# ygjwd12345/UCD

Measured on AMD Instinct MI355X. Metric: images/sec (whole node) per UCD train step, VOC 15-5 step-1, 513^2 bs=24, higher is better.
Workload: dtype bf16

## Files before the change

### include/ucd_hip.h

```cpp
#ifndef UCD_HIP_H
#define UCD_HIP_H

#include <stddef.h>
#include <stdint.h>

#ifdef __cplusplus
extern "C" {
#endif

#define UCD_VERSION 100

typedef void* ucd_stream_t;
typedef void* ucd_comm_t;

enum ucd_dtype { UCD_F32 = 0, UCD_BF16 = 1 };
enum ucd_act { UCD_ACT_IDENTITY = 0, UCD_ACT_LEAKY_RELU = 1, UCD_ACT_ELU = 2  };
#define UCD_ACT_MASK 0xff
#define UCD_NORM_ABS_GAMMA 0x100
enum ucd_pixcon_precision { UCD_PIXCON_F32 = 0, UCD_PIXCON_F16 = 1, UCD_PIXCON_F16_SPLIT = 2 };
enum ucd_error {
  UCD_OK = 0,
  UCD_EINVAL = -1,
  UCD_EALIGN = -2,
  UCD_EWORKSPACE = -3,
// ... 193 lines not shown
                            const int32_t* anchor_pix, const ucd_pixcon_meta* meta,
                            const float* grad_scale, void* d_f_n, int ld_d, int dtype, int BHW, int N,
                            ucd_stream_t stream);

enum ucd_seg_form {
  UCD_SEG_PK_16_8 = 1,
  UCD_SEG_PK_20_4 = 2,
  UCD_SEG_PK_12_12 = 3,
  UCD_SEG_REG_24_16 = 4,
  UCD_SEG_REG_24_24 = 5,
  UCD_SEG_WIDE_FIXED = 6,
  UCD_SEG_WIDE_F32 = 7
};
int ucd_seg_losses_plan(int H, int W, int h, int w, int Ctot, int K, int has_teacher, int d_sem_aligned, int pk, int* form,
                        int* ny, int* nx, size_t* lds_bytes);
size_t ucd_seg_losses_workspace_bytes(int B, int H, int W);
int ucd_seg_losses(const float* sem_s, int ld_s, const float* sem_t, int ld_t, const int64_t* labels,
                   int B, int H, int W, int h, int w, int Ctot, int K, int ignore_index,
                   float ce_weight, float kd_weight, float* loss_out, float* d_sem, int ld_d,
                   void* workspace, size_t workspace_bytes, ucd_stream_t stream);

enum ucd_seg_kd_mode { UCD_KD_UNBIASED = 0, UCD_KD_PLAIN = 1 };
int ucd_seg_losses_plan_ex(int H, int W, int h, int w, int Ctot, int K, int ce_old_cl, int kd_mode, int has_teacher,
                           int d_sem_aligned, int pk, int* form, int* ny, int* nx, size_t* lds_bytes);
int ucd_seg_losses_ex(const float* sem_s, int ld_s, const float* sem_t, int ld_t, const int64_t* labels,
                      int B, int H, int W, int h, int w, int Ctot, int K, int ce_old_cl, int kd_mode, float alpha,
                      int ignore_index, float ce_weight, float kd_weight, float* loss_out, float* d_sem, int ld_d,
                      void* workspace, size_t workspace_bytes, ucd_stream_t stream);

int ucd_seg_confusion(const float* sem, int ld_s, const int64_t* labels, int B, int H, int W, int h, int w, int Ctot,
                      int n_classes, int64_t* hist, int64_t* pred, ucd_stream_t stream);

int ucd_label_path(const uint8_t* const* src, const int* desc, int B, int S, const uint8_t* lut, int* tables,
                   int64_t* out, ucd_stream_t stream);

int ucd_image_path(const uint8_t* const* src, const int* desc, int B, int S, int kmax, int hmax, float mean_r, float mean_g,
                   float mean_b, float std_r, float std_g, float std_b, int* coeff_ws, uint8_t* tmp, float* out,
                   ucd_stream_t stream);

typedef struct ucd_conv1x1_desc {
  const void* a;  int lda;
  const void* w;  int ldw;
  void* y;        int ldy;
  int M, N, K;
  const float* in_mean;  const float* in_scale;  const float* in_shift;  int in_act;  float in_slope;
  int out_mode;
  const float* out_mean;  const float* out_scale;  const float* out_shift;  const float* out_invstd;
  const void* residual;  int ldr;
  int out_act;  float out_slope;
  float* partial;
  int accumulate;
  int taps, H, W, dilation;
  const void* side2;  int ld2;
  int stride;
  float* stat_acc;  const float* stat_shift;  float* stat_acc2;
  int stat_rep;
} ucd_conv1x1_desc;

int ucd_conv1x1_row_tiles(int M);
int ucd_conv1x1_stat_replicas(int M);
size_t ucd_conv1x1_stats_partial_bytes(int M, int C);
int ucd_conv1x1(const ucd_conv1x1_desc* desc, ucd_stream_t stream);

int ucd_conv1x1_stats_finalize(const float* partial, int M, int C, const float* weight, float* running_mean,
                               float* running_var, float momentum, float eps, float* buf, float* pack, int flags,
                               ucd_stream_t stream);

int ucd_abn_reduce_partials(const float* partial, int tiles, int C, float* sums, float* sums_copy, const float* weight,
                            int flags, ucd_stream_t stream);

size_t ucd_conv1x1_wgrad_workspace_bytes(int M, int N, int K);
int ucd_conv1x1_wgrad(const void* dy, int ld_dy, const void* a, int lda, int M, int N, int K,
                      const float* in_mean, const float* in_scale, const float* in_shift, int in_act, float in_slope,
                      void* dw, void* workspace, size_t workspace_bytes, ucd_stream_t stream);

int ucd_abn_sync_finalize(const float* gathered, int world, int M, int C, const float* weight, float* running_mean,
                          float* running_var, float momentum, float eps, float* buf, int flags, ucd_stream_t stream);

int ucd_stem_conv7x7(const float* x, long long sb, long long sc, long long sh, long long sw, int B, int H, int W, const void* w,
                     void* z, ucd_stream_t stream);

int ucd_stem_conv_pool(const float* x, long long sb, long long sc, long long sh, long long sw, int B, int H, int W, const void* w,
                       const float* mean, const float* scale, const float* beta, int act, float slope, void* out, ucd_stream_t stream);
int ucd_stem_pooled_size(int n);
size_t ucd_stem_pool_workspace_bytes(int C);
int ucd_stem_apply_pool(const void* z, int B, int H, int W, int C, const float* mean, const float* scale, const float* beta, int act,
                        float slope, void* out, uint8_t* idx, ucd_stream_t stream);
int ucd_stem_pool_backward(const void* z, const void* dpool, const uint8_t* idx, int B, int H, int W, int C, const float* mean,
                           const float* invstd, const float* scale, const float* beta, const float* weight, float* sums, float count,
                           int act, float slope, void* dz, void* workspace, size_t workspace_bytes, int phase, ucd_stream_t stream);

size_t ucd_conv_wgrad_workspace_bytes(int M, int N, int K, int taps);
int ucd_conv_wgrad(const void* dz, int ld_dz, const void* x, int ld_x, int M, int N, int K, int taps, int H, int W, int dilation,
                   void* dw, float* dw32, int accumulate32, void* workspace, size_t workspace_bytes, ucd_stream_t stream);
int ucd_conv_wgrad_strided(const void* dz, int ld_dz, const void* x, int ld_x, int M, int N, int K, int taps, int H, int W,
                           int dilation, int stride, void* dw, float* dw32, int accumulate32, void* workspace, size_t workspace_bytes,
                           ucd_stream_t stream);
int ucd_conv_wgrad_ex(const void* dz, int ld_dz, const void* x, int ld_x, int M, int N, int K, int taps, int H, int W, int dilation,
                      int stride, void* dw, float* dw32, int accumulate32, void* workspace, size_t workspace_bytes, int flags,
                      ucd_stream_t stream);
int ucd_conv_wgrad_defer(int mode);
int ucd_conv_wgrad_mode(void);
int ucd_conv_wgrad_flush(ucd_stream_t stream);
int ucd_conv_wgrad_drop(ucd_stream_t stream);
int ucd_conv_wgrad_drop_all(void);

int ucd_flip_weights_batched(const void* src_flat, void* dst_flat, const int* blocks, int n_blocks, const long long* entries,
                             ucd_stream_t stream);
int ucd_flip_weights_batched64(const void* src_flat, void* dst_flat, const int* blocks, int n_blocks, const long long* entries,
                               ucd_stream_t stream);

int ucd_transpose_bf16(const void* src, int rows, int cols, void* dst, ucd_stream_t stream);

int ucd_conv_f32(const float* a, int lda, const float* w, int ldw, float* y, int ldy, int M, int N, int K, int taps, int H, int W,
                 int dilation, int accumulate, ucd_stream_t stream);
size_t ucd_conv_f32_wgrad_workspace_bytes(int M, int N, int K, int taps);
int ucd_conv_f32_wgrad(const float* dz, int ld_dz, const float* x, int ld_x, int M, int N, int K, int taps, int H, int W,
                       int dilation, float* dw, void* workspace, size_t workspace_bytes, ucd_stream_t stream);

#define UCD_SGD_MAX_GROUPS 8
typedef struct ucd_sgd_tensor {
  float* p;  const float* g;  float* m;  void* w16;
  long long n;
  int group;  int pad;
} ucd_sgd_tensor;
typedef struct ucd_sgd_hyper {
  double lr[UCD_SGD_MAX_GROUPS], momentum[UCD_SGD_MAX_GROUPS], weight_decay[UCD_SGD_MAX_GROUPS];
  int nesterov[UCD_SGD_MAX_GROUPS];
} ucd_sgd_hyper;
int ucd_sgd_chunk(void);
int ucd_sgd_step(const ucd_sgd_tensor* table, const int* blocks, int n_blocks, const ucd_sgd_hyper* hyper, ucd_stream_t stream);
int ucd_sgd_hyper_store(ucd_sgd_hyper* device_hyper, const ucd_sgd_hyper* hyper, ucd_stream_t stream);
int ucd_sgd_step_dev(const ucd_sgd_tensor* table, const int* blocks, int n_blocks, const ucd_sgd_hyper* device_hyper,
                     ucd_stream_t stream);

#define UCD_REG_EWC 0
#define UCD_REG_PI 1
#define UCD_REG_RW 2
typedef struct ucd_reg_tensor {
  float* p;  float* g;  const float* p_old;  const float* omega;
  float* fisher;  float* score;  float* temp;
  long long n;
  int penalize;  int pad;
} ucd_reg_tensor;
typedef struct ucd_reg_hyper {
  double reg_importance;
  float alpha, one_minus_alpha, lambda_f;
  int iterations;
  int counter;
  int pad;
} ucd_reg_hyper;
int ucd_reg_chunk(void);
int ucd_reg_hyper_store(ucd_reg_hyper* device_hyper, const ucd_reg_hyper* hyper, ucd_stream_t stream);
int ucd_reg_step(const ucd_reg_tensor* table, const int* blocks, int n_blocks, int method, ucd_reg_hyper* device_hyper,
                 double* partials, float* penalty, ucd_stream_t stream);

#ifdef __cplusplus
}
#endif
#endif
```

### ucd_amd/backbone.py

```python
from __future__ import annotations

import sys
from collections import OrderedDict
from functools import partial

import torch
import torch.nn as nn

from . import switches as _switches
from .blocks import Conv2d, ResidualBlock, try_index

_STAGE_DILATION = {16: (1, 1, 1, 2), 8: (1, 1, 2, 4)}


class GlobalAvgPool2d(nn.Module):

    def forward(self, inputs):
        return inputs.flatten(2).mean(dim=2)


class ResNet(nn.Module):
    def __init__(self, structure, bottleneck, norm_act=nn.BatchNorm2d, classes=0,
                 output_stride=16, keep_outputs=False):
        super().__init__()
        if len(structure) != 4:
            raise ValueError("Expected a structure with four values")
        if output_stride not in _STAGE_DILATION:
            raise ValueError("Output stride must be 8 or 16")
        self.structure, self.bottleneck, self.keep_outputs = structure, bottleneck, keep_outputs
        self.dilation = dilation = list(_STAGE_DILATION[output_stride])

        stem = [("conv1", Conv2d(3, 64, 7, stride=2, padding=3, bias=False)), ("bn1", norm_act(64))]
        if try_index(dilation, 0) == 1:
            stem.append(("pool1", nn.MaxPool2d(3, stride=2, padding=1)))
        self.mod1 = nn.Sequential(OrderedDict(stem))

        width = (64, 64, 256) if bottleneck else (64, 64)
        cin = 64
        for stage, depth in enumerate(structure):
            d = try_index(dilation, stage)
            blocks = OrderedDict()
            for b in range(depth):
                stride = 2 if (d == 1 and b == 0 and stage > 0) else 1
                blocks[f"block{b + 1}"] = ResidualBlock(cin, width, norm_act=norm_act, stride=stride, dilation=d)
                cin = width[-1]
            self.add_module(f"mod{stage + 2}", nn.Sequential(blocks))
            width = tuple(2 * c for c in width)
        self.out_channels = cin

        if classes != 0:
            self.classifier = nn.Sequential(OrderedDict(
                [("avg_pool", GlobalAvgPool2d()), ("fc", nn.Linear(cin, classes))]))

    def _stem(self, x):
        m = self.mod1
        if hasattr(m, "pool1") and getattr(m.bn1, "ucd_fused_abn", False) and x.is_cuda:
            pool = m.pool1
            if (pool.kernel_size, pool.stride, pool.padding, pool.dilation, pool.ceil_mode) == (3, 2, 1, 1, False):
                from .abn import stem_norm_pool
                y = _stem_eval_fused(m.conv1, m.bn1, x)
                if y is not None:
                    return y
                z = _stem_conv(m.conv1, x)
                y = stem_norm_pool(m.bn1, z)
                return y if y is not None else pool(m.bn1(z))
        return m(x)

    def forward(self, x):
        outs = [self._stem(x)]
        for name in ("mod2", "mod3", "mod4", "mod5"):
            outs.append(getattr(self, name)(outs[-1]))
        if hasattr(self, "classifier"):
            outs.append(self.classifier(outs[-1]))
        return outs if self.keep_outputs else outs[-1]


class _StemConvFunction(torch.autograd.Function):

    @staticmethod
    def forward(ctx, x, w):
        from . import hip
        ctx.save_for_backward(x, w)
        return hip.stem_conv7x7(x, w)

    @staticmethod
    def backward(ctx, dz):
        x, w = ctx.saved_tensors
        dw = None
        if ctx.needs_input_grad[1]:
            xb = x.to(torch.bfloat16).contiguous(memory_format=torch.channels_last)
            dw = torch.ops.aten.convolution_backward(dz.contiguous(memory_format=torch.channels_last), xb, w, None, [2, 2], [3, 3],
                                                     [1, 1], False, [0, 0], 1, [False, True, False])[1]
        return None, dw


def _stem_conv(conv, x):
    w = conv.working_weight() if hasattr(conv, "working_weight") else None
    if w is None and x.is_cuda and torch.is_autocast_enabled() and torch.get_autocast_dtype("cuda") == torch.bfloat16:
        w = conv.weight.to(torch.bfloat16)
    if (w is None or not x.is_cuda or x.dim() != 4 or x.dtype != torch.float32 or x.requires_grad or conv.bias is not None
            or tuple(conv.weight.shape) != (64, 3, 7, 7) or conv.stride != (2, 2) or conv.padding != (3, 3)
            or conv.dilation != (1, 1) or w.dtype != torch.bfloat16 or not w.is_contiguous(memory_format=torch.channels_last)
            or _switches.get("UCD_OWN_STEM", "1") == "0"):
        return conv(x)
    if torch.is_grad_enabled() and w.requires_grad:
        return _StemConvFunction.apply(x, w)
    from . import hip
    return hip.stem_conv7x7(x, w)


def _stem_eval_fused(conv, bn, x):
    from . import abn as _abn
    if (torch.is_grad_enabled() or bn.training or _switches.get("UCD_STEM_EVAL_FUSED", "1") == "0" or _switches.get("UCD_OWN_STEM", "1") == "0"
            or _switches.get("UCD_STEM_FOLD", "1") == "0" or not getattr(bn, "ucd_fused_abn", False)
            or bn.activation not in ("leaky_relu", "identity")):
        return None
    w = conv.working_weight() if hasattr(conv, "working_weight") else None
    if w is None and x.is_cuda and torch.is_autocast_enabled() and torch.get_autocast_dtype("cuda") == torch.bfloat16:
        w = conv.weight.to(torch.bfloat16)
    if (w is None or not x.is_cuda or x.dim() != 4 or x.dtype != torch.float32 or conv.bias is not None
            or tuple(conv.weight.shape) != (64, 3, 7, 7) or conv.stride != (2, 2) or conv.padding != (3, 3) or conv.dilation != (1, 1)
            or w.dtype != torch.bfloat16 or not w.is_contiguous(memory_format=torch.channels_last) or x.shape[2] < 8 or x.shape[3] < 8):
        return None
    from . import hip
    invstd, scale = bn._eval_constants()
    return hip.stem_conv_pool(x, w, bn.running_mean, scale, bn.bias, _abn._act_code(bn.activation), bn.activation_param)


_NETS = {
    "18": ([2, 2, 2, 2], False), "34": ([3, 4, 6, 3], False), "50": ([3, 4, 6, 3], True),
    "101": ([3, 4, 23, 3], True), "152": ([3, 8, 36, 3], True),
}
__all__ = ["ResNet"]
for _n, (_s, _b) in _NETS.items():
    setattr(sys.modules[__name__], f"net_resnet{_n}", partial(ResNet, structure=_s, bottleneck=_b))
    __all__.append(f"net_resnet{_n}")
```

### ucd_amd/csrc/stem.hip

```cpp
#include "common.h"

namespace ucd {
namespace {

typedef __hip_bfloat16 bf16;
constexpr int kThreads = 256;
constexpr int kRedBlocks = 1024;
constexpr int kApplyRows = 4;

__device__ __forceinline__ float leaky(float z, float slope) { return z > 0.f ? z : z * slope; }
__device__ __forceinline__ float bf16_round(float v) { return __bfloat162float(__float2bfloat16(v)); }

struct StemArgs {
  const bf16* z; int B, H, W, C, PH, PW;
  const float *mean, *scale, *beta, *invstd, *weight, *sums;
  float slope, inv_count;
  int abs_gamma, cg_shift;
};

__global__ __launch_bounds__(kThreads) void stem_apply_pool_kernel(StemArgs p, bf16* __restrict__ out, uint8_t* __restrict__ idx) {
  const int cgs = p.cg_shift, CG = 1 << cgs;
  const int t = blockIdx.x * kThreads + threadIdx.x;
  const int cg = t & (CG - 1), pw = t >> cgs, ph = blockIdx.y, b = blockIdx.z;
  if (pw >= p.PW) return;
// ... 360 lines not shown
    if (tid < kSIP) {
#pragma unroll
      for (int r = 0; r < kSIR; ++r) {
        const bf16 v = __float2bfloat16((premask >> r) & 1u ? pre[r] : 0.f);
        In[r * kSIP + tid] = *reinterpret_cast<const unsigned short*>(&v);
      }
    }
    __syncthreads();
    if (tile + (int)gridDim.x < p.ntiles) fetch(tile + gridDim.x);
    f32x16 acc[2][2];
#pragma unroll
    for (int a = 0; a < 2; ++a)
#pragma unroll
      for (int c = 0; c < 2; ++c)
#pragma unroll
        for (int r = 0; r < 16; ++r) acc[a][c][r] = 0.f;
#pragma unroll
    for (int s = 0; s < kSK / 16; ++s) {
      const int t0 = 2 * s, t1 = 2 * s + 1;
      const int ky = h ? (t1 / 3 > 6 ? 6 : t1 / 3) : t0 / 3, j0 = h ? 8 * (t1 % 3) : 8 * (t0 % 3);
      bf16x8 wf[2], pf[2];
#pragma unroll
      for (int c = 0; c < 2; ++c) wf[c] = *reinterpret_cast<const bf16x8*>(&Wl[(c * 32 + col) * kSWP + 16 * s + 8 * h]);
#pragma unroll
      for (int a = 0; a < 2; ++a) {
        const int orow = wave * 2 + a;
        const unsigned* src = reinterpret_cast<const unsigned*>(&In[(2 * orow + ky) * kSIP + 6 * col + j0]);
        union { unsigned u[4]; bf16x8 v; } f;
        f.u[0] = src[0]; f.u[1] = src[1]; f.u[2] = src[2]; f.u[3] = src[3];
        pf[a] = f.v;
      }
#pragma unroll
      for (int a = 0; a < 2; ++a)
#pragma unroll
        for (int c = 0; c < 2; ++c) acc[a][c] = __builtin_amdgcn_mfma_f32_32x32x16_bf16(wf[c], pf[a], acc[a][c], 0, 0, 0);
    }
    const int ox = ox0 + col;
#pragma unroll
    for (int a = 0; a < 2; ++a) {
      const int orow = wave * 2 + a, oy = oy0 + orow;
      const bool inside = (unsigned)oy < (unsigned)p.OH && (unsigned)ox < (unsigned)p.OW;
      unsigned short* dst = Tl + (orow * kSTW + col) * kFTP;
#pragma unroll
      for (int c = 0; c < 2; ++c)
#pragma unroll
        for (int g = 0; g < 4; ++g) {
          const int ch = c * 32 + 8 * g + 4 * h;
          const float4 mu = *reinterpret_cast<const float4*>(Pl + ch), sc = *reinterpret_cast<const float4*>(Pl + 64 + ch);
          const float4 sh = *reinterpret_cast<const float4*>(Pl + 128 + ch);
          const float m4[4] = {mu.x, mu.y, mu.z, mu.w}, s4[4] = {sc.x, sc.y, sc.z, sc.w}, b4[4] = {sh.x, sh.y, sh.z, sh.w};
          union { bf16 v[4]; uint2 u; } o;
#pragma unroll
          for (int e = 0; e < 4; ++e) {
            const float zq = bf16_round(acc[a][c][g * 4 + e]);
            o.v[e] = __float2bfloat16(leaky((zq - m4[e]) * s4[e] + b4[e], q.slope));
          }
          if (!inside) o.u = make_uint2(0xFF80FF80u, 0xFF80FF80u);
          *reinterpret_cast<uint2*>(dst + ch) = o.u;
        }
    }
    __syncthreads();
    for (int i = tid; i < kFPH * kFPW * 8; i += kThreads) {
      const int cg = i & 7, pp = i >> 3, pr = pp / kFPW, pc = pp - pr * kFPW;
      const int ph = (oy0 + 1) / 2 + pr, pw = (ox0 + 1) / 2 + pc;
      if (ph >= q.PH || pw >= q.PW) continue;
      float best[8];
#pragma unroll
      for (int e = 0; e < 8; ++e) best[e] = -INFINITY;
#pragma unroll
      for (int kh = 0; kh < 3; ++kh)
#pragma unroll
        for (int kw = 0; kw < 3; ++kw) {
          Vec<bf16> v;
          v.raw = *reinterpret_cast<const uint4*>(Tl + ((2 * pr + kh) * kSTW + 2 * pc + kw) * kFTP + cg * 8);
#pragma unroll
          for (int e = 0; e < 8; ++e) best[e] = fmaxf(best[e], v.get(e));
        }
      Vec<bf16> o;
#pragma unroll
      for (int e = 0; e < 8; ++e) o.set(e, best[e]);
      o.store(q.out + (((size_t)b * q.PH + ph) * q.PW + pw) * 64 + cg * 8);
    }
  }
}

bool stem_args_ok(const void* z, int B, int H, int W, int C) {
  return z && B > 0 && B < 65536 && H > 1 && H < 65536 && W > 1 && C >= 8 && (C & (C - 1)) == 0 && C <= 2048 && aligned16(z);
}

}
}

using namespace ucd;

extern "C" {

int ucd_stem_pooled_size(int n) { return (n + 2 - 3) / 2 + 1; }

size_t ucd_stem_pool_workspace_bytes(int C) { return (size_t)kRedBlocks * 2 * C * sizeof(float); }

int ucd_stem_apply_pool(const void* z, int B, int H, int W, int C, const float* mean, const float* scale, const float* beta, int act,
                        float slope, void* out, uint8_t* idx, ucd_stream_t stream) {
  static const char* fn = "ucd_stem_apply_pool";
  UCD_REQUIRE(stem_args_ok(z, B, H, W, C) && mean && scale && out && aligned16(out) && (!idx || (reinterpret_cast<uintptr_t>(idx) & 7) == 0),
              UCD_EINVAL, "%s: dense channels-last bf16 maps with a power-of-two channel count in 8..2048 expected", fn);
  const int a = act & UCD_ACT_MASK;
  UCD_REQUIRE(a != UCD_ACT_ELU, UCD_EUNSUPPORTED, "%s: leaky_relu / identity only (an elu stem keeps the separate passes)", fn);
  StemArgs p{};
  p.z = (const bf16*)z; p.B = B; p.H = H; p.W = W; p.C = C; p.PH = ucd_stem_pooled_size(H); p.PW = ucd_stem_pooled_size(W);
  p.mean = mean; p.scale = scale; p.beta = beta; p.slope = a == UCD_ACT_IDENTITY ? 1.f : slope;
  p.cg_shift = __builtin_ctz(C / 8);
  stem_apply_pool_kernel<<<dim3(ceil_div(p.PW * (C / 8), kThreads), p.PH, B), kThreads, 0, (hipStream_t)stream>>>(p, (bf16*)out, idx);
  return check_launch(fn);
}

int ucd_stem_conv7x7(const float* x, long long sb, long long sc, long long sh, long long sw, int B, int H, int W, const void* w,
                     void* z, ucd_stream_t stream) {
  static const char* fn = "ucd_stem_conv7x7";
  UCD_REQUIRE(x && w && z && B > 0 && H > 0 && W > 0 && aligned16(z) && (reinterpret_cast<uintptr_t>(w) & 1) == 0, UCD_EINVAL,
              "%s: bad arguments", fn);
  StemConvArgs p{};
  p.x = x; p.sb = sb; p.sc = sc; p.sh = sh; p.sw = sw; p.w = (const bf16*)w; p.z = (bf16*)z;
  p.B = B; p.H = H; p.W = W; p.OH = (H + 6 - 7) / 2 + 1; p.OW = (W + 6 - 7) / 2 + 1;
  p.tiles_y = ceil_div(p.OH, kSTH); p.tiles_x = ceil_div(p.OW, kSTW); p.ntiles = B * p.tiles_y * p.tiles_x;
  const int grid = p.ntiles < 768 ? p.ntiles : 768;
  stem_conv7x7_kernel<<<grid, kThreads, 0, (hipStream_t)stream>>>(p);
  return check_launch(fn);
}

int ucd_stem_conv_pool(const float* x, long long sb, long long sc, long long sh, long long sw, int B, int H, int W, const void* w,
                       const float* mean, const float* scale, const float* beta, int act, float slope, void* out, ucd_stream_t stream) {
  static const char* fn = "ucd_stem_conv_pool";
  UCD_REQUIRE(x && w && out && mean && scale && B > 0 && H > 0 && W > 0 && aligned16(out) && (reinterpret_cast<uintptr_t>(w) & 1) == 0 &&
              aligned16(mean) && aligned16(scale) && (!beta || aligned16(beta)), UCD_EINVAL, "%s: bad arguments", fn);
  const int a = act & UCD_ACT_MASK;
  UCD_REQUIRE(a != UCD_ACT_ELU && !(act & UCD_NORM_ABS_GAMMA), UCD_EUNSUPPORTED, "%s: leaky_relu / identity with given scale only", fn);
  StemFusedArgs q{};
  StemConvArgs& p = q.c;
  p.x = x; p.sb = sb; p.sc = sc; p.sh = sh; p.sw = sw; p.w = (const bf16*)w; p.z = nullptr;
  p.B = B; p.H = H; p.W = W; p.OH = (H + 6 - 7) / 2 + 1; p.OW = (W + 6 - 7) / 2 + 1;
  q.PH = ucd_stem_pooled_size(p.OH); q.PW = ucd_stem_pooled_size(p.OW);
  p.tiles_y = ceil_div(q.PH, kFPH); p.tiles_x = ceil_div(q.PW, kFPW); p.ntiles = B * p.tiles_y * p.tiles_x;
  q.mean = mean; q.scale = scale; q.beta = beta; q.slope = a == UCD_ACT_IDENTITY ? 1.f : slope; q.out = (bf16*)out;
  const size_t lds = (size_t)(64 * kSWP + kSIR * kSIP + kSTH * kSTW * kFTP) * 2 + 3 * 64 * 4;
  UCD_TRY_LDS(stem_conv_pool_kernel, 80 * 1024);
  const int grid = p.ntiles < 512 ? p.ntiles : 512;
  stem_conv_pool_kernel<<<grid, kThreads, lds, (hipStream_t)stream>>>(q);
  return check_launch(fn);
}

int ucd_stem_pool_backward(const void* z, const void* dpool, const uint8_t* idx, int B, int H, int W, int C, const float* mean,
                           const float* invstd, const float* scale, const float* beta, const float* weight, float* sums, float count,
                           int act, float slope, void* dz, void* workspace, size_t workspace_bytes, int phase, ucd_stream_t stream) {
  static const char* fn = "ucd_stem_pool_backward";
  UCD_REQUIRE(stem_args_ok(z, B, H, W, C) && dpool && idx && mean && invstd && scale && sums && aligned16(dpool), UCD_EINVAL,
              "%s: bad arguments", fn);
  UCD_REQUIRE(phase >= 1 && phase <= 3 && (!(phase & 2) || (dz && aligned16(dz) && count > 0.f)), UCD_EINVAL, "%s: bad phase / dz", fn);
  const int a = act & UCD_ACT_MASK;
  UCD_REQUIRE(a != UCD_ACT_ELU, UCD_EUNSUPPORTED, "%s: leaky_relu / identity only", fn);
  StemArgs p{};
  p.z = (const bf16*)z; p.B = B; p.H = H; p.W = W; p.C = C; p.PH = ucd_stem_pooled_size(H); p.PW = ucd_stem_pooled_size(W);
  p.mean = mean; p.scale = scale; p.beta = beta; p.invstd = invstd; p.weight = weight; p.sums = sums;
  p.slope = a == UCD_ACT_IDENTITY ? 1.f : slope; p.abs_gamma = (act & UCD_NORM_ABS_GAMMA) != 0;
  p.cg_shift = __builtin_ctz(C / 8);
  hipStream_t s = (hipStream_t)stream;
  if (phase & 1) {
    UCD_REQUIRE(workspace && workspace_bytes >= ucd_stem_pool_workspace_bytes(C), UCD_EWORKSPACE, "%s: workspace too small", fn);
    stem_pool_bwd_reduce_kernel<<<kRedBlocks, kThreads, kThreads * 16 * sizeof(float), s>>>(p, (const bf16*)dpool, idx, (float*)workspace);
    int rc = check_launch(fn);
    if (rc) return rc;
    stem_sum_partials_kernel<<<2 * C, kThreads, 0, s>>>((const float*)workspace, kRedBlocks, C, p.abs_gamma ? weight : nullptr, sums);
    rc = check_launch(fn);
    if (rc) return rc;
  }
  if (phase & 2) {
    p.inv_count = 1.f / count;
    stem_pool_bwd_apply_kernel<<<dim3(ceil_div(((W + 1) / 2) * (C / 8), kThreads), ceil_div(H, kApplyRows), B), kThreads, 0, s>>>(p, (const bf16*)dpool, idx, (bf16*)dz);
    return check_launch(fn);
  }
  return 0;
}

}
```

### ucd_amd/hip.py

```python
from __future__ import annotations

import ctypes as C
import os

import torch

_HERE = os.path.dirname(os.path.abspath(__file__))
LIB_PATH = os.path.join(_HERE, "libucd_hip.so")

F32, BF16 = 0, 1
ACT_IDENTITY, ACT_LEAKY_RELU, ACT_ELU = 0, 1, 2
ACT_CODES = {"identity": ACT_IDENTITY, "leaky_relu": ACT_LEAKY_RELU, "elu": ACT_ELU}
ACT_MASK = 0xFF
NORM_ABS_GAMMA = 0x100
PIX_TILE = 128
PIXCON_LD = 256
PIXCON_F32, PIXCON_F16, PIXCON_F16_SPLIT = 0, 1, 2
KD_UNBIASED, KD_PLAIN = 0, 1
SEG_FORMS = {1: "pk<16,8>", 2: "pk<20,4>", 3: "pk<12,12>", 4: "reg<24,16>", 5: "reg<24,24>", 6: "wide/fixed", 7: "wide/f32"}
PIXCON_PATHS = {1: "f32", 2: "f32/wide", 3: "f16/planned", 4: "f16/split"}
PIXCON_PRECISION = {"f32": PIXCON_F32, "fp32": PIXCON_F32, "f16": PIXCON_F16, "fp16": PIXCON_F16,
                    "f16_split": PIXCON_F16_SPLIT}


# ... 12 lines not shown
    _fields_ = [("a", C.c_void_p), ("lda", C.c_int), ("w", C.c_void_p), ("ldw", C.c_int), ("y", C.c_void_p), ("ldy", C.c_int),
                ("M", C.c_int), ("N", C.c_int), ("K", C.c_int),
                ("in_mean", C.c_void_p), ("in_scale", C.c_void_p), ("in_shift", C.c_void_p), ("in_act", C.c_int),
                ("in_slope", C.c_float), ("out_mode", C.c_int),
                ("out_mean", C.c_void_p), ("out_scale", C.c_void_p), ("out_shift", C.c_void_p), ("out_invstd", C.c_void_p),
                ("residual", C.c_void_p), ("ldr", C.c_int), ("out_act", C.c_int), ("out_slope", C.c_float),
                ("partial", C.c_void_p), ("accumulate", C.c_int),
                ("taps", C.c_int), ("H", C.c_int), ("W", C.c_int), ("dilation", C.c_int),
                ("side2", C.c_void_p), ("ld2", C.c_int), ("stride", C.c_int),
                ("stat_acc", C.c_void_p), ("stat_shift", C.c_void_p), ("stat_acc2", C.c_void_p), ("stat_rep", C.c_int)]


_p, _i, _f, _z = C.c_void_p, C.c_int, C.c_float, C.c_size_t
SIGNATURES = {
    "ucd_version": (_i, []),
    "ucd_last_error": (C.c_char_p, []),
    "ucd_abn_workspace_bytes": (_z, [_i, _i]),
    "ucd_abn_stats": (_i, [_p, _i, _i, _i, _i, _p, _i, _p, _p, _p, _z, _p]),
    "ucd_abn_stats_finalize": (_i, [_p, _i, _i, _i, _i, _p, _i, _p, _p, _p, _p, _p, _f, _f, _p, _p, _p, _i, _p, _z, _p]),
    "ucd_abn_finalize": (_i, [_p, _p, _f, _i, _p, _p, _p, _f, _f, _p, _p, _p, _i, _p]),
    "ucd_abn_eval_params": (_i, [_p, _p, _f, _i, _p, _p, _i, _p]),
    "ucd_abn_apply": (_i, [_p, _i, _p, _i, _p, _i, _i, _i, _i, _p, _i, _p, _p, _p, _i, _f, _p]),
    "ucd_conv1x1_stat_replicas": (_i, [_i]),
    "ucd_fill_zero": (_i, [_p, _z, _p]),
    "ucd_abn_apply_stats": (_i, [_p, _i, _p, _i, _p, _i, _i, _i, _p, _i, _p, _f, _p, _p, _p, _p, _f, _f, _p, _p, _p, _i, _f, _p]),
    "ucd_abn_bwd_apply_raw": (_i, [_p, _i, _p, _i, _p, _i, _p, _i, _p, _i, _i, _i, _p, _p, _p, _p, _p, _p, _p, _i, _p, _f, _i, _f, _p]),
    "ucd_abn_bwd_reduce": (_i, [_p, _i, _p, _i, _p, _i, _i, _i, _i, _p, _i, _p, _p, _p, _p, _p, _i, _f, _p, _p, _z, _p]),
    "ucd_label_path": (_i, [_p, _p, _i, _i, _p, _p, _p, _p]),
    "ucd_image_path": (_i, [_p, _p, _i, _i, _i, _i, _f, _f, _f, _f, _f, _f, _p, _p, _p, _p]),
    "ucd_gemm_load": (_i, [C.c_char_p]),
    "ucd_gemm_workspace_bytes": (_z, []),
    "ucd_gemm_bf16": (_i, [_i, _i, _i, _i, _p, _i, _p, _i, _p, _i, _p, _z, _i, _p]),
    "ucd_gemm_bf16_acc": (_i, [_i, _i, _i, _i, _p, _i, _p, _i, _p, _i, _p, _z, _p]),
    "ucd_gemm_has_plan": (_i, [_i, _i, _i, _i, _i, _i, _i]),
    "ucd_gemm_last_tuned_us": (_f, []),
    "ucd_gemm_last_candidates": (_i, []),
    "ucd_comm_load": (_i, [C.c_char_p]),
    "ucd_comm_unique_id": (_i, [_p, _z]),
    "ucd_comm_init": (_i, [_p, _z, _i, _i, C.POINTER(C.c_void_p)]),
    "ucd_comm_destroy": (_i, [_p]),
    "ucd_comm_all_gather": (_i, [_p, _p, _p, _z, _p]),
    "ucd_comm_all_reduce_sum": (_i, [_p, _p, _z, _p]),
    "ucd_comm_init_local": (_i, [_i, _i, C.POINTER(C.c_void_p)]),
    "ucd_comm_ipc_handle_bytes": (_z, []),
    "ucd_comm_ipc_create": (_i, [_p, _i, _i, _p]),
    "ucd_comm_ipc_connect": (_i, [_p, _p]),
    "ucd_comm_ipc_drop": (_i, [_p]),
    "ucd_comm_ipc_timeouts": (C.c_uint, [_p]),
    "ucd_abn_sync_forward_comm": (_i, [_p, _i, _p, _i, _p, _i, _p, _i, _i, _i, _i, _p, _i, _p, _p, _p, _p, _f, _f, _p, _i, _f,
                                       _p, _z, _p]),
    "ucd_abn_sync_backward_comm": (_i, [_p, _i, _p, _i, _p, _i, _p, _i, _p, _i, _p, _i, _i, _i, _i, _p, _i, _p, _p, _p, _p, _p,
                                        _p, _p, _i, _f, _p, _z, _p]),
    "ucd_abn_sync_stats": (_i, [_p, _i, _i, _i, _i, _p, _i, _p, _p, _p, _p, _z, _p]),
    "ucd_abn_sync_forward": (_i, [_p, _i, _p, _i, _p, _i, _i, _i, _i, _p, _i, _p, _i, _p, _p, _p, _p, _f, _f, _p, _i, _f, _p]),
    "ucd_abn_sync_bwd_reduce": (_i, [_p, _i, _p, _i, _p, _i, _i, _i, _i, _p, _i, _p, _p, _p, _p, _p, _i, _f, _p, _p, _p, _z, _p]),
    "ucd_abn_bwd_apply": (_i, [_p, _i, _p, _i, _p, _i, _p, _i, _p, _i, _i, _i, _i, _p, _i, _p, _p, _p, _p, _p, _p,
                               _f, _i, _i, _f, _p]),
    "ucd_abn_forward": (_i, [_p, _i, _p, _i, _p, _i, _i, _i, _i, _p, _i, _p, _p, _p, _p, _f, _f, _i, _p, _p, _i, _f, _p, _z, _p]),
    "ucd_abn_backward": (_i, [_p, _i, _p, _i, _p, _i, _p, _i, _p, _i, _i, _i, _i, _p, _i, _p, _p, _p, _p, _p, _p, _f, _i, _i,
                              _i, _f, _p, _z, _p]),
    "ucd_plane_sum": (_i, [_p, _i, _i, _i, _i, _i, _f, _p, _p]),
    "ucd_window_mean_workspace_bytes": (_z, [_i, _i, _i, _i, _i]),
    "ucd_window_mean": (_i, [_p, _i, _i, _i, _i, _i, _i, _i, _i, _p, _i, _p, _z, _p]),
    "ucd_attmap_workspace_bytes": (_z, [_i, _i]),
    "ucd_attmap": (_i, [_p, _i, _p, _i, _i, _i, _i, _i, _p, _z, _p]),
    "ucd_attn_mse_workspace_bytes": (_z, [_i, _i]),
    "ucd_attn_mse": (_i, [_p, _i, _p, _i, _i, _i, _i, _i, _f, _p, _p, _i, _p, _z, _p]),
    "ucd_conv1x1_row_tiles": (_i, [_i]),
    "ucd_conv1x1_stats_partial_bytes": (_z, [_i, _i]),
    "ucd_conv1x1": (_i, [C.POINTER(Conv1x1Desc), _p]),
    "ucd_conv1x1_stats_finalize": (_i, [_p, _i, _i, _p, _p, _p, _f, _f, _p, _p, _i, _p]),
    "ucd_abn_reduce_partials": (_i, [_p, _i, _i, _p, _p, _p, _i, _p]),
    "ucd_conv1x1_wgrad_workspace_bytes": (_z, [_i, _i, _i]),
    "ucd_conv1x1_wgrad": (_i, [_p, _i, _p, _i, _i, _i, _i, _p, _p, _p, _i, _f, _p, _p, _z, _p]),
    "ucd_abn_sync_finalize": (_i, [_p, _i, _i, _i, _p, _p, _p, _f, _f, _p, _i, _p]),
    "ucd_stem_pooled_size": (_i, [_i]),
    "ucd_stem_pool_workspace_bytes": (_z, [_i]),
    "ucd_stem_apply_pool": (_i, [_p, _i, _i, _i, _i, _p, _p, _p, _i, _f, _p, _p, _p]),
    "ucd_stem_pool_backward": (_i, [_p, _p, _p, _i, _i, _i, _i, _p, _p, _p, _p, _p, _p, _f, _i, _f, _p, _p, _z, _i, _p]),
    "ucd_conv_wgrad_workspace_bytes": (_z, [_i, _i, _i, _i]),
    "ucd_conv_wgrad": (_i, [_p, _i, _p, _i, _i, _i, _i, _i, _i, _i, _i, _p, _p, _i, _p, _z, _p]),
    "ucd_stem_conv7x7": (_i, [_p, C.c_longlong, C.c_longlong, C.c_longlong, C.c_longlong, _i, _i, _i, _p, _p, _p]),
    "ucd_stem_conv_pool": (_i, [_p, C.c_longlong, C.c_longlong, C.c_longlong, C.c_longlong, _i, _i, _i, _p, _p, _p, _p, _i, _f, _p, _p]),
    "ucd_conv_wgrad_strided": (_i, [_p, _i, _p, _i, _i, _i, _i, _i, _i, _i, _i, _i, _p, _p, _i, _p, _z, _p]),
    "ucd_conv_wgrad_ex": (_i, [_p, _i, _p, _i, _i, _i, _i, _i, _i, _i, _i, _i, _p, _p, _i, _p, _z, _i, _p]),
    "ucd_conv_wgrad_defer": (_i, [_i]),
    "ucd_conv_wgrad_mode": (_i, []),
    "ucd_conv_wgrad_flush": (_i, [_p]),
    "ucd_conv_wgrad_drop": (_i, [_p]),
    "ucd_conv_wgrad_drop_all": (_i, []),
    "ucd_transpose_bf16": (_i, [_p, _i, _i, _p, _p]),
    "ucd_conv_f32": (_i, [_p, _i, _p, _i, _p, _i, _i, _i, _i, _i, _i, _i, _i, _i, _p]),
    "ucd_conv_f32_wgrad_workspace_bytes": (_z, [_i, _i, _i, _i]),
    "ucd_conv_f32_wgrad": (_i, [_p, _i, _p, _i, _i, _i, _i, _i, _i, _i, _i, _p, _p, _z, _p]),
    "ucd_flip_weights_batched": (_i, [_p, _p, _p, _i, _p, _p]),
    "ucd_flip_weights_batched64": (_i, [_p, _p, _p, _i, _p, _p]),
    "ucd_sgd_chunk": (_i, []),
    "ucd_sgd_step": (_i, [_p, _p, _i, _p, _p]),
    "ucd_sgd_hyper_store": (_i, [_p, _p, _p]),
    "ucd_sgd_step_dev": (_i, [_p, _p, _i, _p, _p]),
    "ucd_reg_chunk": (_i, []),
    "ucd_reg_hyper_store": (_i, [_p, _p, _p]),
    "ucd_reg_step": (_i, [_p, _p, _i, _i, _p, _p, _p, _p]),
    "ucd_pixcon_prep_workspace_bytes": (_z, [_i, _i]),
    "ucd_pixcon_prep": (_i, [_p, _i, _i, _i, _i, _i, _i, _p, _i, _i, _i, _i, _p, _p, _p, _p, _p, _p, _z, _p]),
    "ucd_pixcon_gather": (_i, [_p, _i, _p, _i, _i, _i, _i, _p, _p, _p, _i, _p, _p, _i, _p, _i, _p, _p, _p, _p]),
    "ucd_pixcon_loss_workspace_bytes": (_z, [_i, _i, _i]),
    "ucd_pixcon_loss_plan": (_i, [_i, _i, _i, _i, _f, _p, _p, _p, _p, _p, _p, _p]),
    "ucd_pixcon_loss": (_i, [_p, _i, _i, _p, _p, _i, _i, _p, _p, _i, _p, _i, _f, _i, _i, _p, _p, _i, _p, _p, _z, _p]),
    "ucd_pixcon_loss_given_p": (_i, [_p, _i, _i, _p, _p, _i, _p, _i, _f, _i, _p, _p, _i, _p, _p, _z, _p]),
    "ucd_pixcon_scatter_grad": (_i, [_p, _p, _i, _p, _p, _p, _p, _p, _i, _i, _i, _i, _p]),
    "ucd_seg_confusion": (_i, [_p, _i, _p, _i, _i, _i, _i, _i, _i, _i, _p, _p, _p]),
    "ucd_seg_losses_workspace_bytes": (_z, [_i, _i, _i]),
    "ucd_seg_losses_plan": (_i, [_i, _i, _i, _i, _i, _i, _i, _i, _i, _p, _p, _p, _p]),
    "ucd_seg_losses": (_i, [_p, _i, _p, _i, _p, _i, _i, _i, _i, _i, _i, _i, _i, _f, _f, _p, _p, _i, _p, _z, _p]),
    "ucd_seg_losses_plan_ex": (_i, [_i, _i, _i, _i, _i, _i, _i, _i, _i, _i, _i, _p, _p, _p, _p]),
    "ucd_seg_losses_ex": (_i, [_p, _i, _p, _i, _p, _i, _i, _i, _i, _i, _i, _i, _i, _i, _f, _i, _f, _f, _p, _p, _i, _p, _z, _p]),
}

_lib = None


def load():
    global _lib
    if _lib is None:
        if not os.path.exists(LIB_PATH):
            raise ImportError(
                f"{LIB_PATH} not found: build the HIP kernels first (python -c 'import __graft_entry__ as g; "
                f"g.build()' or make -C ucd_amd/csrc).  ucd_amd has no CPU fallback.")
        lib = C.CDLL(LIB_PATH)
        for name, (res, args) in SIGNATURES.items():
            fn = getattr(lib, name)
            fn.restype, fn.argtypes = res, args
        _lib = lib
    return _lib


def _check(rc, name):
    if rc != 0:
        msg = load().ucd_last_error().decode(errors="replace")
        raise RuntimeError(f"{name} failed (code {rc}): {msg}")


_timing = None


def enable_call_timing():
    global _timing
    _timing = {}
    return _timing


def disable_call_timing():
    global _timing
    _timing = None


class _Timed:

    def __init__(self, name, work, flops=None, staged=None):
        self.name, self.work, self.flops, self.staged = name, work, flops, staged

    def __enter__(self):
        self.start = torch.cuda.Event(enable_timing=True)
        self.end = torch.cuda.Event(enable_timing=True)
        self.start.record(torch.cuda.current_stream())
# ... 332 lines not shown
    if conv3 is not None:
        d.taps, d.H, d.W, d.dilation = 9, int(conv3[0]), int(conv3[1]), int(conv3[2])
        if len(conv3) > 3:
            d.stride = int(conv3[3])
    elif strided is not None:
        d.H, d.W, d.stride = int(strided[0]), int(strided[1]), int(strided[2])
    if in_norm is not None:
        mean, scale, shift, act, slope = in_norm
        d.in_mean, d.in_scale, d.in_shift, d.in_act, d.in_slope = ptr(mean), ptr(scale), ptr(shift), act & ACT_MASK, slope
    d.out_mode = out_mode
    if out_norm is not None:
        mean, scale, shift, invstd, act, slope = out_norm
        d.out_mean, d.out_scale, d.out_shift, d.out_invstd = ptr(mean), ptr(scale), ptr(shift), ptr(invstd)
        d.out_act, d.out_slope = act & ACT_MASK, slope
    if residual is not None:
        d.residual, d.ldr = residual.data_ptr(), residual.stride(0)
    if side2 is not None:
        d.side2, d.ld2 = side2.data_ptr(), side2.stride(0)
    d.partial = ptr(partial)
    d.accumulate = 1 if accumulate else 0
    d.stat_acc, d.stat_shift, d.stat_acc2, d.stat_rep = ptr(stat_acc), ptr(stat_shift), ptr(stat_acc2), int(stat_rep)
    work = 2 * M * 9 * K * N if conv3 is not None else 2 * (M * K + M * N * (1 + (residual is not None) + bool(accumulate)
                                                                                 + (side2 is not None)))
    bn = 128 if (N % 128 == 0 and ((M + 127) // 128) * (N // 128) > 128) else 64
    staged = 2 * M * N * K * (9 if conv3 is not None else 1) * (1.0 / 128 + 1.0 / bn)
    with _timed("ucd_conv3x3" if conv3 is not None else "ucd_conv1x1", work, None if conv3 is not None else 2 * M * K * N, staged):
        _check(lib.ucd_conv1x1(C.byref(d), stream()), "ucd_conv1x1")
    return y


def abn_apply_stats(x, y, residual, M, Cc, acc, kshift, count, weight, bias, running_mean, running_var, momentum, eps, buf, act,
                    slope, reps=1):
    with _timed("ucd_abn_apply", M * Cc * x.element_size() * (2 + (residual is not None))):
        _check(load().ucd_abn_apply_stats(ptr(x), Cc, ptr(y), Cc, ptr(residual), Cc if residual is not None else 0, M, Cc, ptr(acc),
                                          int(reps), ptr(kshift), float(count), ptr(weight), ptr(bias), ptr(running_mean), ptr(running_var),
                                          float(momentum), float(eps), ptr(buf[3 * Cc:]), ptr(buf[4 * Cc:]), ptr(buf[5 * Cc:]), act,
                                          float(slope), stream()), "ucd_abn_apply_stats")
    return y


def abn_bwd_apply_raw(x, dy, y, dx, dz, M, Cc, mean, invstd, scale, shift, weight, sums, grad_sums, grad_out, count, act, slope,
                      reps=1):
    with _timed("ucd_abn_bwd_apply", M * Cc * x.element_size() * (3 + (y is not None) + (dz is not None))):
        _check(load().ucd_abn_bwd_apply_raw(ptr(x), Cc, ptr(dy), Cc, ptr(y), Cc if y is not None else 0, ptr(dx), Cc, ptr(dz),
                                            Cc if dz is not None else 0, M, Cc, ptr(mean), ptr(invstd), ptr(scale), ptr(shift),
                                            ptr(weight), ptr(sums), ptr(grad_sums), int(reps), ptr(grad_out), float(count), act, float(slope),
                                            stream()), "ucd_abn_bwd_apply_raw")
    return dx


def conv1x1_wgrad(dy, a, dw, in_norm=None):
    lib = load()
    M, N = dy.shape
    K = a.shape[1]
    nbytes = lib.ucd_conv1x1_wgrad_workspace_bytes(M, N, K)
    ws = workspace(nbytes, dy.device, "wgrad")
    mean = scale = shift = None
    act, slope = ACT_IDENTITY, 1.0
    if in_norm is not None:
        mean, scale, shift, act, slope = in_norm
    with _timed("ucd_conv1x1_wgrad", 2 * (M * N + M * K)):
        _check(lib.ucd_conv1x1_wgrad(ptr(dy), dy.stride(0), ptr(a), a.stride(0), M, N, K, ptr(mean), ptr(scale), ptr(shift),
                                     act & ACT_MASK, float(slope), ptr(dw), ptr(ws), nbytes, stream()), "ucd_conv1x1_wgrad")
    return dw


def abn_sync_finalize(gathered, world, M, Cc, weight, running_mean, running_var, momentum, eps, buf, flags=0):
    _check(load().ucd_abn_sync_finalize(ptr(gathered), world, M, Cc, ptr(weight), ptr(running_mean), ptr(running_var),
                                        float(momentum), float(eps), ptr(buf), int(flags) & NORM_ABS_GAMMA, stream()),
           "ucd_abn_sync_finalize")


def stem_conv7x7(x, w):
    lib = load()
    B, Cc, H, W = x.shape
    OH, OW = (H - 1) // 2 + 1, (W - 1) // 2 + 1
    z = torch.empty((B, 64, OH, OW), dtype=torch.bfloat16, device=x.device, memory_format=torch.channels_last)
    sb, sc, sh, sw = x.stride()
    with _timed("ucd_stem_conv7x7", x.numel() * 4 + z.numel() * 2):
        _check(lib.ucd_stem_conv7x7(ptr(x), sb, sc, sh, sw, B, H, W, ptr(w), ptr(z), stream()), "ucd_stem_conv7x7")
    return z


def stem_conv_pool(x, w, mean, scale, beta, act, slope):
    lib = load()
    B, _, H, W = x.shape
    OH, OW = (H + 6 - 7) // 2 + 1, (W + 6 - 7) // 2 + 1
    PH, PW = lib.ucd_stem_pooled_size(OH), lib.ucd_stem_pooled_size(OW)
    out = torch.empty((B, 64, PH, PW), dtype=torch.bfloat16, device=x.device, memory_format=torch.channels_last)
    sb, sc, sh, sw = x.stride()
    with _timed("ucd_stem_conv7x7", x.numel() * 4 + out.numel() * 2):
        _check(lib.ucd_stem_conv_pool(ptr(x), sb, sc, sh, sw, B, H, W, ptr(w), ptr(mean), ptr(scale), ptr(beta), act, float(slope),
                                      ptr(out), stream()), "ucd_stem_conv_pool")
    return out


def stem_apply_pool(z, mean, scale, beta, act, slope, want_idx):
    lib = load()
    B, Cc, H, W = z.shape
    PH, PW = lib.ucd_stem_pooled_size(H), lib.ucd_stem_pooled_size(W)
    out = torch.empty((B, Cc, PH, PW), dtype=z.dtype, device=z.device, memory_format=torch.channels_last)
    idx = torch.empty((B, PH, PW, Cc), dtype=torch.uint8, device=z.device) if want_idx else None
    with _timed("ucd_stem_apply_pool", (z.numel() + out.numel()) * 2 + (idx.numel() if idx is not None else 0)):
        _check(lib.ucd_stem_apply_pool(ptr(z), B, H, W, Cc, ptr(mean), ptr(scale), ptr(beta), act, float(slope), ptr(out), ptr(idx),
                                       stream()), "ucd_stem_apply_pool")
    return out, idx


def stem_pool_backward(z, dpool, idx, mean, invstd, scale, beta, weight, sums, count, act, slope, dz, phase):
    lib = load()
    B, Cc, H, W = z.shape
    nbytes = lib.ucd_stem_pool_workspace_bytes(Cc)
    ws = workspace(nbytes, z.device)
    work = (z.numel() * (2 if phase & 1 else 0) + (2 * z.numel() * 2 if phase & 2 else 0) + dpool.numel() * 3 * (1 + (phase == 3)))
    with _timed("ucd_stem_pool_backward", work):
        _check(lib.ucd_stem_pool_backward(ptr(z), ptr(dpool), ptr(idx), B, H, W, Cc, ptr(mean), ptr(invstd), ptr(scale), ptr(beta),
                                          ptr(weight), ptr(sums), float(count), act, float(slope), ptr(dz), ptr(ws), nbytes,
                                          int(phase), stream()), "ucd_stem_pool_backward")


def wgrad_defer(mode):
    return int(load().ucd_conv_wgrad_defer(int(mode) & 3))


def _wgrad_side_release(stream=None):
    from . import abn as _abn
    node = _abn._abn_node()
    if node is not None:
        node.wgrad_side_release(stream)


def wgrad_flush():
    s = stream()
    _check(load().ucd_conv_wgrad_flush(s), "ucd_conv_wgrad_flush")
    _wgrad_side_release(s)


def wgrad_drop():
    s = stream()
    rc = load().ucd_conv_wgrad_drop(s)
    if rc == 0:
        _wgrad_side_release(s)
    return rc


def wgrad_drop_all():
    rc = load().ucd_conv_wgrad_drop_all()
    if rc == 0:
        _wgrad_side_release()
    return rc


_wgrad_turn = {}


def conv_wgrad(dz, x, dw=None, conv3=None, dw32=None, accumulate32=False, strided=None, defer=False, side=False):
    lib = load()
    M, N = dz.shape
    K = x.shape[1]
    taps = 9 if conv3 is not None else 1
    H, W, d = (int(conv3[0]), int(conv3[1]), int(conv3[2])) if conv3 is not None else (0, 0, 1)
    stride = 1
    if conv3 is not None and len(conv3) > 3:
        stride = int(conv3[3])
    elif strided is not None:
        H, W, stride = int(strided[0]), int(strided[1]), int(strided[2])
# ... 73 lines not shown
```

### ucd_amd/switches.py

```python
from __future__ import annotations

import os

DEFAULTS = {
    "UCD_FUSED_CONV1X1": "1",
    "UCD_BWD_LINK": "1",
    "UCD_BLOCK_LINK": "1",
    "UCD_PROJ_ALIAS": "1",
    "UCD_DGRAD_VIA_FWD": "1",
    "UCD_LIB_GEMM_WIDE": "0",
    "UCD_OWN3X3_MIN_TILES": "1",
    "UCD_OWN3X3_WIDE": "1",
    "UCD_OWN_STRIDED": "1",
    "UCD_OWN_WGRAD": "1",
    "UCD_F32_OWN_CONV": "0",
    "UCD_OWN_HEADS": "1",
    "UCD_OWN_STEM": "1",
    "UCD_WGRAD3": "1",
    "UCD_CONV_PIPE": "auto",
    "UCD_CONV_BN64_TILES": "128",
    "UCD_CONV_LW64_TILES": "128",
    "UCD_WGRAD_DEFER": "1",
    "UCD_WGRAD_STREAM": "1",
    "UCD_CONV3_MIN_ROWS": "0",
    "UCD_STAT_ATOMIC": "1",
    "UCD_SEG_PK": "1",
    "UCD_SEG_KD_EX": "1",
    "UCD_FUSED_LDE": "1",
    "UCD_STEM_EVAL_FUSED": "1",
    "UCD_STEM_FOLD": "1",
    "UCD_ABN_NODE": "1",
    "UCD_ABN_GENERIC": "0",
    "UCD_SGD": "hip",
    "UCD_STEP_GRAPH": "auto",
    "UCD_TEACHER_OVERLAP": "1",
    "UCD_DIRECT_RCCL": "1",
    "UCD_IPC_SYNC": "auto",
    "UCD_IPC_TIMEOUT_MS": "60000",
    "UCD_DDP_LATE_COPY": "1",
    "UCD_DDP_DIRECT": "auto",
    "UCD_FORCE_COLLECTIVES": "0",
}

_cache: dict = {}


def get(name: str, default: str | None = None) -> str:
    v = _cache.get(name)
    if v is None:
        if default is None:
            default = DEFAULTS.get(name, "")
        v = _cache[name] = os.environ.get(name, default)
    return v


def set(name: str, value) -> None:
    os.environ[name] = str(value)
    _cache[name] = str(value)


def unset(name: str) -> None:
    os.environ.pop(name, None)
    _cache.pop(name, None)


def reload() -> None:
    _cache.clear()


def snapshot() -> dict:
    return {k: get(k) for k in DEFAULTS}
```

Baseline: 864.7.

## Add custom MFMA kernel for stem 7x7 conv weight gradient

Replaces the aten convolution_backward weight-gradient path for the 7x7 stride-2 stem conv with a dedicated HIP kernel. The kernel reads the fp32 input directly and converts it to bf16 in LDS, which avoids a separate cast and channels_last copy. It also prefetches the next tile into registers and accumulates with 32x32x16 bf16 MFMA, writing per-block partial slabs that a second kernel reduces. The cost is an extra reduction launch, a workspace of up to 512 fp32 slabs, and a hand-written fragment layout that could be wrong.

New measurement: 869.2, median of 6. Within noise of the previous version (+0.5%).

```diff
diff --git a/include/ucd_hip.h b/include/ucd_hip.h
--- a/include/ucd_hip.h
+++ b/include/ucd_hip.h
@@ -299,6 +299,9 @@
 
 int ucd_stem_conv_pool(const float* x, long long sb, long long sc, long long sh, long long sw, int B, int H, int W, const void* w,
                        const float* mean, const float* scale, const float* beta, int act, float slope, void* out, ucd_stream_t stream);
+size_t ucd_stem_conv7x7_wgrad_workspace_bytes(int B, int H, int W);
+int ucd_stem_conv7x7_wgrad(const float* x, long long sb, long long sc, long long sh, long long sw, int B, int H, int W, const void* dz,
+                           void* dw, float* dw32, int accumulate32, void* workspace, size_t workspace_bytes, ucd_stream_t stream);
 int ucd_stem_pooled_size(int n);
 size_t ucd_stem_pool_workspace_bytes(int C);
 int ucd_stem_apply_pool(const void* z, int B, int H, int W, int C, const float* mean, const float* scale, const float* beta, int act,
diff --git a/ucd_amd/backbone.py b/ucd_amd/backbone.py
--- a/ucd_amd/backbone.py
+++ b/ucd_amd/backbone.py
@@ -87,7 +87,10 @@
     def backward(ctx, dz):
         x, w = ctx.saved_tensors
         dw = None
-        if ctx.needs_input_grad[1]:
+        if ctx.needs_input_grad[1] and _switches.get("UCD_OWN_STEM_WGRAD", "1") != "0":
+            from . import hip
+            dw = hip.stem_conv7x7_wgrad(x, dz.contiguous(memory_format=torch.channels_last))
+        elif ctx.needs_input_grad[1]:
             xb = x.to(torch.bfloat16).contiguous(memory_format=torch.channels_last)
             dw = torch.ops.aten.convolution_backward(dz.contiguous(memory_format=torch.channels_last), xb, w, None, [2, 2], [3, 3],
                                                      [1, 1], False, [0, 0], 1, [False, True, False])[1]
diff --git a/ucd_amd/csrc/stem.hip b/ucd_amd/csrc/stem.hip
--- a/ucd_amd/csrc/stem.hip
+++ b/ucd_amd/csrc/stem.hip
@@ -466,6 +466,137 @@
       o.store(q.out + (((size_t)b * q.PH + ph) * q.PW + pw) * 64 + cg * 8);
     }
   }
+}
+
+constexpr int kWIP = 280;
+constexpr int kWDP = 96;
+constexpr int kWOut = 64 * 147;
+constexpr int kWMaxSlabs = 512;
+
+struct StemWgradArgs {
+  const float* x; long long sb, sc, sh, sw;
+  const bf16* dz;
+  float* slabs;
+  int B, H, W, OH, OW, tiles_y, tiles_x, ntiles;
+};
+
+typedef short s16x4 __attribute__((ext_vector_type(4)));
+__device__ __forceinline__ s16x4 lds_read_tr(const unsigned short* p) {
+  return __builtin_amdgcn_ds_read_tr16_b64_v4i16((__attribute__((address_space(3))) s16x4*)p);
+}
+
+__global__ __launch_bounds__(kThreads, 2) void stem_conv7x7_wgrad_kernel(StemWgradArgs p) {
+  typedef float f32x16 __attribute__((ext_vector_type(16)));
+  typedef __bf16 bf16x8 __attribute__((ext_vector_type(8)));
+  union Frag { s16x4 h[2]; bf16x8 v; };
+  __shared__ __attribute__((aligned(16))) unsigned short Dl[kSTH * kSTW * kWDP];
+  __shared__ __attribute__((aligned(16))) unsigned short In[kSIR * kWIP];
+  const int tid = threadIdx.x, lane = tid & 63, wave = tid >> 6;
+  for (int i = tid; i < kSIR * kWIP; i += kThreads) In[i] = 0;
+  const int fe = tid < 210 ? tid : 209, fpx = fe / 3, fc = fe - fpx * 3;
+  const int dcol = tid >> 3, dcg = tid & 7;
+  float pre[kSIR];
+  uint4 dpre[kSTH];
+  auto origin = [&](int tile, int& b, int& oy0, int& ox0) {
+    b = tile / (p.tiles_y * p.tiles_x);
+    const int rem = tile - b * p.tiles_y * p.tiles_x;
+    oy0 = (rem / p.tiles_x) * kSTH; ox0 = (rem % p.tiles_x) * kSTW;
+  };
+  auto fetch = [&](int tile) {
+    int b, oy0, ox0;
+    origin(tile, b, oy0, ox0);
+    const int ix = 2 * ox0 - 3 + fpx;
+    const bool colok = fpx < 2 * kSTW + 5 && (unsigned)ix < (unsigned)p.W;
+    const float* src = p.x + b * p.sb + fc * p.sc + (colok ? ix : 0) * p.sw;
+#pragma unroll
+    for (int r = 0; r < kSIR; ++r) {
+      const int iy = 2 * oy0 - 3 + r;
+      const bool ok = colok && (unsigned)iy < (unsigned)p.H;
+      const float v = src[(ok ? iy : 0) * p.sh];
+      pre[r] = ok ? v : 0.f;
+    }
+    const int ox = ox0 + dcol;
+    const bf16* dsrc = p.dz + ((size_t)b * p.OH * p.OW + min(ox, p.OW - 1)) * 64 + dcg * 8;
+#pragma unroll
+    for (int r = 0; r < kSTH; ++r) {
+      const int oy = oy0 + r;
+      const uint4 v = *reinterpret_cast<const uint4*>(dsrc + (size_t)min(oy, p.OH - 1) * p.OW * 64);
+      dpre[r] = (ox < p.OW && oy < p.OH) ? v : make_uint4(0u, 0u, 0u, 0u);
+    }
+  };
+  const int h = lane >> 5, g = (lane >> 4) & 1, q = (lane & 15) >> 2, pp = lane & 3;
+  const int nblk = wave & 1, ky0 = (wave >> 1) * 4, row = 4 * h + q;
+  const unsigned short* abase = Dl + row * kWDP + nblk * 32 + 16 * g + 4 * pp;
+  const unsigned short* bbase[4];
+#pragma unroll
+  for (int j = 0; j < 4; ++j) bbase[j] = In + min(ky0 + j, 6) * kWIP + (2 * row + 4 * g + pp) * 4;
+  f32x16 acc[4];
+#pragma unroll
+  for (int j = 0; j < 4; ++j)
+#pragma unroll
+    for (int r = 0; r < 16; ++r) acc[j][r] = 0.f;
+
+  fetch(blockIdx.x);
+  for (int tile = blockIdx.x; tile < p.ntiles; tile += gridDim.x) {
+    __syncthreads();
+    if (tid < 210) {
+#pragma unroll
+      for (int r = 0; r < kSIR; ++r) {
+        const bf16 v = __float2bfloat16(pre[r]);
+        In[r * kWIP + fpx * 4 + fc] = *reinterpret_cast<const unsigned short*>(&v);
+      }
+    }
+#pragma unroll
+    for (int r = 0; r < kSTH; ++r) *reinterpret_cast<uint4*>(&Dl[(r * kSTW + dcol) * kWDP + dcg * 8]) = dpre[r];
+    __syncthreads();
+    if (tile + (int)gridDim.x < p.ntiles) fetch(tile + gridDim.x);
+#pragma unroll
+    for (int orow = 0; orow < kSTH; ++orow)
+#pragma unroll
+      for (int s = 0; s < 2; ++s) {
+        Frag a, b[4];
+        const unsigned short* ap = abase + (orow * kSTW + 16 * s) * kWDP;
+        a.h[0] = lds_read_tr(ap); a.h[1] = lds_read_tr(ap + 8 * kWDP);
+#pragma unroll
+        for (int j = 0; j < 4; ++j) {
+          const unsigned short* bp = bbase[j] + 2 * orow * kWIP + 16 * s * 8;
+          b[j].h[0] = lds_read_tr(bp); b[j].h[1] = lds_read_tr(bp + 8 * 8);
+        }
+#pragma unroll
+        for (int j = 0; j < 4; ++j) acc[j] = __builtin_amdgcn_mfma_f32_32x32x16_bf16(a.v, b[j].v, acc[j], 0, 0, 0);
+      }
+  }
+  const int col = lane & 31, kx = col >> 2, c = col & 3;
+  if (kx < 7 && c < 3) {
+    float* dst = p.slabs + (size_t)blockIdx.x * kWOut + kx * 3 + c;
+#pragma unroll
+    for (int j = 0; j < 4; ++j) {
+      if (ky0 + j > 6) continue;
+#pragma unroll
+      for (int r = 0; r < 16; ++r) {
+        const int n = nblk * 32 + (r & 3) + 8 * (r >> 2) + 4 * h;
+        dst[n * 147 + (ky0 + j) * 21] = acc[j][r];
+      }
+    }
+  }
+}
+
+__global__ __launch_bounds__(kThreads) void stem_wgrad_sum_kernel(const float* __restrict__ slabs, int nslabs, bf16* __restrict__ dw,
+                                                                 float* __restrict__ dw32, int accumulate) {
+  __shared__ float red[8][32];
+  const int o = threadIdx.x & 31, sl = threadIdx.x >> 5, i = blockIdx.x * 32 + o;
+  float s0 = 0.f, s1 = 0.f;
+  int k = sl;
+  for (; k + 8 < nslabs; k += 16) { s0 += slabs[(size_t)k * kWOut + i]; s1 += slabs[(size_t)(k + 8) * kWOut + i]; }
+  if (k < nslabs) s0 += slabs[(size_t)k * kWOut + i];
+  red[sl][o] = s0 + s1;
+  __syncthreads();
+  if (sl) return;
+  float t = red[0][o];
+#pragma unroll
+  for (int l = 1; l < 8; ++l) t += red[l][o];
+  if (dw) dw[i] = __float2bfloat16(t);
+  if (dw32) dw32[i] = accumulate ? dw32[i] + t : t;
 }
 
 bool stem_args_ok(const void* z, int B, int H, int W, int C) {
@@ -530,6 +661,34 @@
   UCD_TRY_LDS(stem_conv_pool_kernel, 80 * 1024);
   const int grid = p.ntiles < 512 ? p.ntiles : 512;
   stem_conv_pool_kernel<<<grid, kThreads, lds, (hipStream_t)stream>>>(q);
+  return check_launch(fn);
+}
+
+size_t ucd_stem_conv7x7_wgrad_workspace_bytes(int B, int H, int W) {
+  if (B <= 0 || H <= 0 || W <= 0) return 0;
+  const long long tiles = (long long)B * ceil_div((H - 1) / 2 + 1, kSTH) * ceil_div((W - 1) / 2 + 1, kSTW);
+  return (size_t)(tiles < kWMaxSlabs ? tiles : kWMaxSlabs) * kWOut * sizeof(float);
+}
+
+int ucd_stem_conv7x7_wgrad(const float* x, long long sb, long long sc, long long sh, long long sw, int B, int H, int W, const void* dz,
+                           void* dw, float* dw32, int accumulate32, void* workspace, size_t workspace_bytes, ucd_stream_t stream) {
+  static const char* fn = "ucd_stem_conv7x7_wgrad";
+  UCD_REQUIRE(x && dz && (dw || dw32) && B > 0 && H > 0 && W > 0 && aligned16(dz) && (reinterpret_cast<uintptr_t>(dw) & 1) == 0 &&
+              (reinterpret_cast<uintptr_t>(dw32) & 3) == 0, UCD_EINVAL, "%s: bad arguments", fn);
+  StemWgradArgs p{};
+  p.x = x; p.sb = sb; p.sc = sc; p.sh = sh; p.sw = sw; p.dz = (const bf16*)dz; p.slabs = (float*)workspace;
+  p.B = B; p.H = H; p.W = W; p.OH = (H + 6 - 7) / 2 + 1; p.OW = (W + 6 - 7) / 2 + 1;
+  p.tiles_y = ceil_div(p.OH, kSTH); p.tiles_x = ceil_div(p.OW, kSTW);
+  const long long tiles = (long long)B * p.tiles_y * p.tiles_x;
+  UCD_REQUIRE(tiles < (1ll << 30), UCD_EINVAL, "%s: too many tiles", fn);
+  p.ntiles = (int)tiles;
+  const int grid = p.ntiles < kWMaxSlabs ? p.ntiles : kWMaxSlabs;
+  UCD_REQUIRE(workspace && (reinterpret_cast<uintptr_t>(workspace) & 3) == 0 &&
+              workspace_bytes >= ucd_stem_conv7x7_wgrad_workspace_bytes(B, H, W), UCD_EWORKSPACE, "%s: workspace too small", fn);
+  stem_conv7x7_wgrad_kernel<<<grid, kThreads, 0, (hipStream_t)stream>>>(p);
+  int rc = check_launch(fn);
+  if (rc) return rc;
+  stem_wgrad_sum_kernel<<<kWOut / 32, kThreads, 0, (hipStream_t)stream>>>((const float*)workspace, grid, (bf16*)dw, dw32, accumulate32);
   return check_launch(fn);
 }
 
diff --git a/ucd_amd/hip.py b/ucd_amd/hip.py
--- a/ucd_amd/hip.py
+++ b/ucd_amd/hip.py
@@ -118,6 +118,8 @@
     "ucd_conv_wgrad": (_i, [_p, _i, _p, _i, _i, _i, _i, _i, _i, _i, _i, _p, _p, _i, _p, _z, _p]),
     "ucd_stem_conv7x7": (_i, [_p, C.c_longlong, C.c_longlong, C.c_longlong, C.c_longlong, _i, _i, _i, _p, _p, _p]),
     "ucd_stem_conv_pool": (_i, [_p, C.c_longlong, C.c_longlong, C.c_longlong, C.c_longlong, _i, _i, _i, _p, _p, _p, _p, _i, _f, _p, _p]),
+    "ucd_stem_conv7x7_wgrad_workspace_bytes": (_z, [_i, _i, _i]),
+    "ucd_stem_conv7x7_wgrad": (_i, [_p, C.c_longlong, C.c_longlong, C.c_longlong, C.c_longlong, _i, _i, _i, _p, _p, _p, _i, _p, _z, _p]),
     "ucd_conv_wgrad_strided": (_i, [_p, _i, _p, _i, _i, _i, _i, _i, _i, _i, _i, _i, _p, _p, _i, _p, _z, _p]),
     "ucd_conv_wgrad_ex": (_i, [_p, _i, _p, _i, _i, _i, _i, _i, _i, _i, _i, _i, _p, _p, _i, _p, _z, _i, _p]),
     "ucd_conv_wgrad_defer": (_i, [_i]),
@@ -616,6 +618,20 @@
     return z
 
 
+def stem_conv7x7_wgrad(x, dz, dw=None, dw32=None, accumulate32=False):
+    lib = load()
+    B, _, H, W = x.shape
+    if dw is None and dw32 is None:
+        dw = torch.empty((64, 3, 7, 7), dtype=torch.bfloat16, device=x.device, memory_format=torch.channels_last)
+    nbytes = lib.ucd_stem_conv7x7_wgrad_workspace_bytes(B, H, W)
+    ws = workspace(nbytes, x.device, "stem_wgrad")
+    sb, sc, sh, sw = x.stride()
+    with _timed("ucd_stem_conv7x7_wgrad", x.numel() * 4 + dz.numel() * 2):
+        _check(lib.ucd_stem_conv7x7_wgrad(ptr(x), sb, sc, sh, sw, B, H, W, ptr(dz), ptr(dw), ptr(dw32), 1 if accumulate32 else 0,
+                                          ptr(ws), nbytes, stream()), "ucd_stem_conv7x7_wgrad")
+    return dw if dw is not None else dw32
+
+
 def stem_conv_pool(x, w, mean, scale, beta, act, slope):
     lib = load()
     B, _, H, W = x.shape
diff --git a/ucd_amd/switches.py b/ucd_amd/switches.py
--- a/ucd_amd/switches.py
+++ b/ucd_amd/switches.py
@@ -16,6 +16,7 @@
     "UCD_F32_OWN_CONV": "0",
     "UCD_OWN_HEADS": "1",
     "UCD_OWN_STEM": "1",
+    "UCD_OWN_STEM_WGRAD": "1",
     "UCD_WGRAD3": "1",
     "UCD_CONV_PIPE": "auto",
     "UCD_CONV_BN64_TILES": "128",
```
